# clovaai/frostnet

Measured on AMD Instinct MI355X. Metric: images/sec FrostNet-Large 224x224 QAT fwd+bwd, higher is better.
Workload: dtype int8; 1 GPU; FrostNet-Large int8 fake-quant QAT fwd+bwd + GradBoost-SGD step (noise on; StatAssist FP epoch is a one-off before it), batch=512/GPU, 224x224 NHWC, qnnpack qconfig v0 (per-tensor); per_gpu_batch=512, global_batch=512, resolution=224, parallelism=dp1, hip_graph=True, grad_dtype=bf16

## Files before the change

frostnet_amd/_lib.py:

```python
import ctypes as C
import os

import torch

_HERE = os.path.dirname(os.path.abspath(__file__))
LIB_PATH = os.environ.get("FROST_HIP_LIB", os.path.join(_HERE, "libfrost_hip.so"))
_lib = None

P, I, L, F, D = C.c_void_p, C.c_int, C.c_int64, C.c_float, C.c_double

Q_MIN, Q_MAX, Q_SCALE, Q_ZP, Q_FQMIN, Q_FQMAX, Q_INV, Q_QMAX, Q_OBS_EN, Q_FQ_EN, Q_STRIDE = 0, 1, 2, 3, 4, 5, 6, 7, 8, 10, 12
COEF_ROWS = int(os.environ.get("FROST_COEF_ROWS_ALLOC", "14"))
COEF_ROWS_NAMED = 8
DWQ_NC, DWQ_SPREAD_MAX = int(os.environ.get("FROST_DWQ_NC", "4")), 32768
COEF_A, COEF_B = 0, 1
COEF_M, COEF_R, COEF_K1, COEF_S1, COEF_S2, COEF_VFRAC = 2, 3, 4, 5, 6, 7
STATS_BYTES_PER_CH = 24 * int(os.environ.get("FROST_STATS_TABLES", "4"))


class FrostWDesc(C.Structure):
    _fields_ = [("w", P), ("gamma", P), ("rvar", P), ("qrec", P), ("wq_pack", P), ("wsum", P), ("minmax2", P),
                ("wt_pack", P), ("wscale", P), ("wmin", P), ("wmax", P), ("cout", C.c_int32), ("cin_g", C.c_int32), ("kk", C.c_int32), ("kind", C.c_int32),
                ("cpad", C.c_int32), ("kpad", C.c_int32), ("reserved0", C.c_int32), ("reserved1", C.c_int32)]

# ... 126 lines not shown
    "frost_dw_conv_fwd": [P, P, P, P, I, I, I, I, I, I, I, P, P, P, I, P, P],
    "frost_stem_im2col": [P, P, I, I, I, P, P],
    "frost_stem_wgrad_remap": [P, I, I, P, P],
    "frost_conv_finalize": [P, L, I, P, P, P, P, P, P, P, I, I, I, P, P, P, P],
    "frost_cat_observe": [P, P, P, I, P],
    "frost_cat_requant": [P, P, I, P, P, I, L, P, P, P],
    "frost_add_minmax": [P, P, P, P, L, P, P],
    "frost_add_minmax_observe": [P, P, P, P, L, P, P, I, P],
    "frost_add_requant": [P, P, P, P, L, P, P, P],
    "frost_avgpool": [P, P, I, I, I, P, P, P],
    "frost_classifier_fwd": [P, P, P, P, I, I, I, P, P, P],
    "frost_pw_conv_bwd": [P, P, P, P, P, P, L, I, I, I, P, P, I, P, P, P, I, P],
    "frost_pw_wgrad": [P, P, P, L, I, I, P, P],
    "frost_pw_bwd_fused_ok": [L, I, I],
    "frost_pw_conv_int": [P, P, P, P, L, I, I, P, P],
    "frost_pw_ew": [P, L, I, P, P, I, I, P, P, P],
    "frost_pw_ew_emit_add": [P, L, I, P, P, I, P, P, P, P, P, I, P],
    "frost_pw_ew_add_bwd": [P, L, I, P, P, I, I, P, P, P, P, P, P, I, P, P],
    "frost_pw_conv_fwd_keep": [P, P, P, P, L, I, I, P, P, P, P],
    "frost_pwc_bwd_ok": [L, I, I],
    "frost_pwc_conv_bwd": [P, P, P, P, L, I, I, I, P, P, I, P, P, P],
    "frost_pwc_conv_fwd_emit": [P, P, P, P, L, I, I, P, P, P, P],
    "frost_block_supported": [I, I, I, I, I, I],
    "frost_block_fwd": [P, P],
    "frost_block_bwd": [P, P, P],
    "frost_block_expand_dw_stats": [P, P, P, P, P, P, P, I, I, I, I, I, P, P, I, P, P, P],
    "frost_block_dw_stats": [P, P, P, P, I, I, I, I, I, P, P, P],
    "frost_block_dw_reduce_supported": [I, I, I, I, I, I],
    "frost_block_dw_bwd_supported": [I, I, I, I, I],
    "frost_block_dw_bwd_reduce": [P, P, P, P, I, I, I, I, I, P, P, I, P, P],
    "frost_block_dw_bwd": [P, P, P, P, P, P, I, I, I, I, I, P, P, I, P, P, P, P],
    "frost_block_dw_bwd_c1": [P, P, P, P, P, P, I, I, I, I, I, P, P, I, P, P, P, P, P, P, P, P, I, I, P],
    "frost_block_dw_bwd_c1_ok": [I, I, I, I, I, I],
    "frost_block_dw_reduce": [P, P, P, P, P, P, I, P, I, I, I, I, I, P, P, I, P, P, P, P],
    "frost_pw_dgrad_wide_ok": [L, I, I],
    "frost_pw_dgrad_wide": [P, P, P, L, I, I, P, I, P],
    "frost_pw_conv_bwd_fused": [P, P, P, P, P, P, L, I, I, P, P, I, P, P, P, I, P, P],
    "frost_dw_conv_bwd": [P, P, P, P, P, I, I, I, I, I, I, I, P, P, I, P, P, P],
    "frost_dw_conv_bwd_dc_wgrad": [P, P, P, P, P, I, I, I, I, I, I, P, P, I, P, P, P, P],
    "frost_dw_dgrad": [P, P, P, I, I, I, I, I, I, P, I, P, P],
    "frost_dw_wgrad": [P, P, P, I, I, I, I, I, I, P, P],
    "frost_dw_bwd_fused_ok": [I, I, I, I, I],
    "frost_dw_bwd_fused": [P, P, P, P, P, P, I, I, I, I, I, I, P, P, I, P, P, P, P],
    "frost_dw_bwd_fused_c1_ok": [I, I, I, I, I, I],
    "frost_dw_bwd_fused_c1": [P, P, P, P, P, P, I, I, I, I, I, I, P, P, I, P, P, P, P, P, P, P, P, I, I, P],
    "frost_weight_grad_finalize": [P, P, P, P, P, P, I, I, I, I, P, P, P, I, P, P],
    "frost_weight_grad_finalize_table": [P, I, P],
    "frost_infer_weight_prep": [P, I, P],
    "frost_infer_stem_im2col": [P, I, I, I, L, L, L, L, P, P],
    "frost_infer_stem_ok": [I],
    "frost_infer_stem": [P, I, I, I, L, L, L, L, P, P, I, I, P, P],
    "frost_infer_pw": [P, P, P, L, I, I, I, P, P],
    "frost_infer_dw": [P, P, P, I, I, I, I, I, I, I, P, P],
    "frost_infer_cat": [P, I, P, I, L, P, P],
    "frost_infer_add": [P, P, L, P, P],
    "frost_infer_avgpool": [P, I, I, I, P, P],
    "frost_linear_f32": [P, P, P, I, I, I, P, P],
    "frost_float_weight_prep": [P, I, P],
    "frost_float_bn_finalize": [P, I, L, P],
    "frost_float_bn_eval": [P, I, P],
    "frost_float_bwd_finalize": [P, I, L, P],
    "frost_float_pw": [P, P, P, L, I, I, I, I, P, I, P, I, P],
    "frost_float_dw": [P, P, I, I, I, I, I, I, I, I, P, P, P],
    "frost_float_ew": [P, P, L, I, I, I, P, I, P, I, P],
    "frost_float_ew_f32": [P, P, L, I, I, I, P, I, P, I, P],
    "frost_float_dw_dgrad": [P, P, I, I, I, I, I, I, P, P],
# ... 65 lines not shown
    "frost_conv_finalize_converted": [P, P, P, P, P, P, I, P, P, P],
    "frost_conv_finalize_converted_fb": [P, P, P, P, P, P, I, P, P, P],
    "frost_add_qnnpack": [P, P, P, P, L, P, P, P],
    "frost_avgpool_q": [P, I, I, I, P, P],
    "frost_cvt_head_ok": [I, I, I, I, I],
    "frost_cvt_head": [P, P, P, P, I, I, I, I, I, I, I, P, L, L, P, L, L, P],
    "frost_cvt_place": [P, P, I, I, I, I, P, L, L, P],
    "frost_stem_converted_ok": [I],
    "frost_stem_converted": [P, I, I, I, L, L, L, L, P, P, P, P, P, I, I, P, P],
    "frost_hswish_fwd": [P, P, L, P, P, P, P, I, P, P, P],
    "frost_hswish_bwd": [P, P, L, P, P, I, P],
    "frost_hswish_converted": [P, P, L, P, P, P, P, P],
    "frost_classifier_q": [P, P, P, P, I, I, I, P, P, P, P],
    "frost_classifier_q_fb": [P, P, P, P, I, I, I, P, P, P, P],
}
SYMBOLS = sorted(list(_PROTOS) + ["frost_last_error"])


def load_library():
    global _lib
    if _lib is not None:
        return _lib
    if not os.path.exists(LIB_PATH):
        raise RuntimeError(f"{LIB_PATH} not found: run `python __graft_entry__.py` (build()) first. "
                           "frostnet_amd has no CPU fallback for the HIP path.")
    lib = C.CDLL(LIB_PATH)
    for name, args in _PROTOS.items():
        fn = getattr(lib, name)
        fn.argtypes = args
        fn.restype = C.c_int
    lib.frost_last_error.restype = C.c_char_p
    lib.frost_g32_scratch_bytes.restype = C.c_int64
    lib.frost_sq_fwd_slot_bytes.restype = C.c_int64
    if lib.frost_abi_version() != ABI_VERSION or lib.frost_ticket_words() != TICKET_WORDS or lib.frost_fin_desc_bytes() != C.sizeof(FrostFinDesc):
        raise RuntimeError(f"{LIB_PATH}: ABI mismatch (library abi {lib.frost_abi_version()} / ticket words {lib.frost_ticket_words()} / FrostFinDesc "
                           f"{lib.frost_fin_desc_bytes()} B, binding {ABI_VERSION} / {TICKET_WORDS} / {C.sizeof(FrostFinDesc)} B): rebuild with `python __graft_entry__.py`")
    if lib.frost_ema_entry_bytes() != C.sizeof(FrostEmaEntry):
        raise RuntimeError(f"{LIB_PATH}: FrostEmaEntry is {lib.frost_ema_entry_bytes()} B in the library, {C.sizeof(FrostEmaEntry)} B in the binding: rebuild with `python __graft_entry__.py`")
    _lib = lib
    return lib


def ptr(t):
    if t is None:
        return None
    return C.c_void_p(t.data_ptr())


def stream():
    return C.c_void_p(torch.cuda.current_stream().cuda_stream)


class Profiler:

    def __init__(self, only=None):
        self.only = only
        self.records = []

    def summary(self):
        torch.cuda.synchronize()
        agg = {}
        for label, nbytes, e0, e1 in self.records:
            a = agg.setdefault(label, [0, 0.0, 0])
            a[0] += 1
            a[1] += e0.elapsed_time(e1)
            a[2] += nbytes
# ... 44 lines not shown
```

frostnet_amd/csrc/frost_block.hip:

```cpp
#include "frost_common.h"

typedef int v2i __attribute__((ext_vector_type(2)));
#include <stdlib.h>

__device__ __forceinline__ int blk_xcd_item(int b, int total, int on) {
  if (!on || b >= (total & ~31)) return b;
  const int xcd = b & 7, j = b >> 3;
  return (j >> 2) * 32 + xcd * 4 + (j & 3);
}
__device__ __forceinline__ int blk_xcd_run(int b, int total, int run) {
  if (run < 2 || b >= total - total % (8 * run)) return b;
  const int xcd = b & 7, j = b >> 3;
  return (j / run) * (8 * run) + xcd * run + (j % run);
}
static int blk_xcd_on() { static const int on = getenv("FROST_BLK_XCD") ? atoi(getenv("FROST_BLK_XCD")) : 1; return on; }

struct BlkAP {
  const int8_t* x; const float* qx;
  const int8_t* w1; const int32_t* wsum1;
  const float* coef1; const float* qy1; int8_t* y1;
  const int8_t* wq2; const int32_t* wsum2;
  uint8_t* stats2; FrostFinDesc fin;
  int n, cin, c, cpad, KS, kstr, nchunk, csplit, imgs, rounds, xrun;
};
// ... 1078 lines not shown
#pragma unroll
  for (int t = 0; t < K * K; ++t) red[(w * K * K + t) * 64 + lane] = (w < G::NRG) ? wacc[t] - zpf * sdc : 0.0f;
  __syncthreads();
  const float sx = p.qx[FROST_Q_SCALE];
  for (int i = tid; i < K * K * 64; i += NT) {
    const int t = i >> 6, l2 = i & 63; const int c2 = chunk * 64 + l2;
    float sum = 0.0f;
#pragma unroll
    for (int w2 = 0; w2 < NW; ++w2) sum += red[(w2 * K * K + t) * 64 + l2];
    if (c2 < p.c) atomicAdd(dwq_dst(p.dwq, (int64_t)p.c * K * K) + (int64_t)c2 * K * K + t, sum * sx);
  }
}

template <int K, int HW, int NW, int KS1 = 0>
static int launch_blk_c(BlkCP& p, hipStream_t s) {
  using G = BlkGeoC<K, HW, NW>;
  if (KS1 > 0) p.c1_kstr = KS1 * 64 + 16;
  const size_t lds = (KS1 > 0) ? (size_t)G::lds_c1(p.c1_kstr, KS1) : (size_t)G::lds();
  FROST_REQUIRE(lds <= 160 * 1024, "block_dw_bwd: LDS budget exceeded");
  static bool attr_set = false; static int occ = 0;
  if (!attr_set) {
    hipFuncSetAttribute((const void*)k_blk_dw_bwd<K, HW, NW, KS1>, hipFuncAttributeMaxDynamicSharedMemorySize, 160 * 1024); attr_set = true;
    if (hipOccupancyMaxActiveBlocksPerMultiprocessor(&occ, (const void*)k_blk_dw_bwd<K, HW, NW, KS1>, NW * 64, lds) != hipSuccess || occ < 1) occ = 1;
  }
  if (p.imgs <= 0) {
    const int rounds = p.rounds > 0 ? p.rounds : 1;
    int groups = (256 * occ * rounds) / p.nchunk; if (groups < 1) groups = 1; if (groups > p.n) groups = p.n;
    p.imgs = (p.n + groups - 1) / groups;
  }
  p.xmap = blk_xcd_on();
  hipLaunchKernelGGL((k_blk_dw_bwd<K, HW, NW, KS1>), dim3((unsigned)(((p.n + p.imgs - 1) / p.imgs) * p.nchunk)), dim3(NW * 64), lds, s, p);
  return frost_check_launch("block_dw_bwd");
}

extern "C" int frost_block_dw_bwd_supported(int h, int w, int k, int stride, int c) {
  return (h == w && (h == 7 || h == 14) && (k == 3 || k == 5) && stride == 1 && (c % 8) == 0) ? 1 : 0;
}

extern "C" int frost_block_dw_bwd_c1_ok(int h, int w, int k, int stride, int c, int c1_cin) {
  static const int on = getenv("FROST_BLK_C1") ? atoi(getenv("FROST_BLK_C1")) : 2;
  const int ks1 = (c1_cin + 63) / 64;
  return (frost_block_dw_bwd_supported(h, w, k, stride, c) && ((on >> (h == 7 ? 0 : 1)) & 1) && (c1_cin % 8) == 0 && ks1 >= 1 && ks1 <= (h == 7 ? 5 : (k == 5 ? 2 : 3))) ? 1 : 0;
}
static int blk_dw_bwd_impl(const int8_t* x, const float* qrec_x, const int8_t* wq_pack, const int32_t* wsum, const float* qrec_w, const float* wscale,
                           int n, int h, int w, int c, int k, const float* coef, const float* qrec_y, int relu, const uint16_t* gout, uint16_t* dx,
                           float* dwq, const int8_t* c1_x, const float* c1_qrec_x, const int8_t* c1_wq_pack, const int32_t* c1_wsum, float* c1_coef, int c1_cin, int c1_relu,
                           void* stream);
extern "C" int frost_block_dw_bwd(const int8_t* x, const float* qrec_x, const int8_t* wq_pack, const int32_t* wsum, const float* qrec_w, const float* wscale,
                                  int n, int h, int w, int c, int k, const float* coef, const float* qrec_y, int relu, const uint16_t* gout, uint16_t* dx,
                                  float* dwq, void* stream) {
  return blk_dw_bwd_impl(x, qrec_x, wq_pack, wsum, qrec_w, wscale, n, h, w, c, k, coef, qrec_y, relu, gout, dx, dwq, nullptr, nullptr, nullptr, nullptr, nullptr, 0, 0, stream);
}
extern "C" int frost_block_dw_bwd_c1(const int8_t* x, const float* qrec_x, const int8_t* wq_pack, const int32_t* wsum, const float* qrec_w, const float* wscale,
                                     int n, int h, int w, int c, int k, const float* coef, const float* qrec_y, int relu, const uint16_t* gout, uint16_t* dx,
                                     float* dwq, const int8_t* c1_x, const float* c1_qrec_x, const int8_t* c1_wq_pack, const int32_t* c1_wsum, float* c1_coef, int c1_cin,
                                     int c1_relu, void* stream) {
  FROST_REQUIRE(c1_x && c1_qrec_x && c1_wq_pack && c1_wsum && c1_coef && dx, "block_dw_bwd_c1: incomplete conv1 arguments (the data gradient is required)");
  FROST_REQUIRE(frost_block_dw_bwd_c1_ok(h, w, k, 1, c, c1_cin), "block_dw_bwd_c1: the conv1 fold has no instance for this shape");
  return blk_dw_bwd_impl(x, qrec_x, wq_pack, wsum, qrec_w, wscale, n, h, w, c, k, coef, qrec_y, relu, gout, dx, dwq, c1_x, c1_qrec_x, c1_wq_pack, c1_wsum, c1_coef, c1_cin, c1_relu, stream);
}
static int blk_dw_bwd_impl(const int8_t* x, const float* qrec_x, const int8_t* wq_pack, const int32_t* wsum, const float* qrec_w, const float* wscale,
                           int n, int h, int w, int c, int k, const float* coef, const float* qrec_y, int relu, const uint16_t* gout, uint16_t* dx,
                           float* dwq, const int8_t* c1_x, const float* c1_qrec_x, const int8_t* c1_wq_pack, const int32_t* c1_wsum, float* c1_coef, int c1_cin, int c1_relu,
                           void* stream) {
  FROST_REQUIRE(frost_block_dw_bwd_supported(h, w, k, 1, c), "block_dw_bwd: unsupported shape (7x7 / 14x14 maps, k in {3,5}, stride 1)");
  FROST_REQUIRE(x && wq_pack && wsum && coef && qrec_y && gout && dwq, "block_dw_bwd: incomplete arguments");
  BlkCP p = {};
  p.c1_x = c1_x; p.c1_qx = c1_qrec_x; p.c1_w = c1_wq_pack; p.c1_wsum = c1_wsum; p.c1_coef = c1_coef; p.c1_cin = c1_cin; p.c1_relu = c1_relu;
  p.x = x; p.qx = qrec_x; p.wq = wq_pack; p.wsum = wsum; p.qw = qrec_w; p.wscale = wscale; p.coef = (float*)coef ; p.qy = qrec_y; p.gout = gout; p.dx = dx; p.dwq = dwq;
  p.n = n; p.c = c; p.cpad = round_up(c, 16); p.nchunk = (c + 63) / 64; p.relu = relu; p.sr = frost_sr_enabled();
  p.inv_count = 1.0f / (float)((int64_t)n * h * w);
  static const int imgs_env = getenv("FROST_BLK_IMGS_C") ? atoi(getenv("FROST_BLK_IMGS_C")) : 0;
  static const int wgs_env = getenv("FROST_BLK_WGS_C") ? atoi(getenv("FROST_BLK_WGS_C")) : 0;
  static const int rounds_env = getenv("FROST_BLK_ROUNDS_C") ? atoi(getenv("FROST_BLK_ROUNDS_C")) : 0;
  int imgs = imgs_env > 0 ? imgs_env : (wgs_env > 0 ? (int)(((int64_t)n * p.nchunk + wgs_env - 1) / wgs_env) : 0);
  if (imgs > n) imgs = n;
  p.imgs = imgs; p.rounds = rounds_env;
  hipStream_t s = as_stream(stream);
  if (c1_x) {
    const int ks1 = (c1_cin + 63) / 64;
#define BLK_C1(KK, HH, NWW, KS) if (k == KK && h == HH && ks1 == KS) return launch_blk_c<KK, HH, NWW, KS>(p, s);
    BLK_C1(5, 7, 4, 1) BLK_C1(5, 7, 4, 2) BLK_C1(5, 7, 4, 3) BLK_C1(5, 7, 4, 4) BLK_C1(5, 7, 4, 5)
    BLK_C1(3, 7, 4, 1) BLK_C1(3, 7, 4, 2) BLK_C1(3, 7, 4, 3) BLK_C1(3, 7, 4, 4) BLK_C1(3, 7, 4, 5)
    BLK_C1(5, 14, 8, 1) BLK_C1(5, 14, 8, 2)
    BLK_C1(3, 14, 8, 1) BLK_C1(3, 14, 8, 2) BLK_C1(3, 14, 8, 3)
#undef BLK_C1
    FROST_REQUIRE(false, "block_dw_bwd_c1: no instance");
  }
  if (h == 7) return (k == 3) ? launch_blk_c<3, 7, 4>(p, s) : launch_blk_c<5, 7, 4>(p, s);
  return (k == 3) ? launch_blk_c<3, 14, 8>(p, s) : launch_blk_c<5, 14, 8>(p, s);
}

template <int K, int HW, int NW>
__global__ __launch_bounds__(NW * 64, 4) void k_blk_dw_bred(const BlkCP p) {
  using G = BlkGeoC<K, HW, NW>;
  constexpr int MAP = G::MAP, PAD = G::PAD, PITCH = G::PITCH, NT = G::NT;
  constexpr int XU = (MAP * 8 + NT - 1) / NT;
  extern __shared__ __attribute__((aligned(16))) uint8_t smem[];
  uint8_t* const xpl = smem;
  uint8_t* const gt = smem + G::PLANE;
  const int tid = threadIdx.x, lane = tid & 63, w = __builtin_amdgcn_readfirstlane(tid >> 6);
  const int bi = blk_xcd_item((int)blockIdx.x, (int)gridDim.x, p.xmap);
  const int chunk = bi % p.nchunk, ig = bi / p.nchunk;
  const int img_lo = ig * p.imgs, img_hi = min(img_lo + p.imgs, p.n);
  const int ch = chunk * 64 + lane; const bool chok = ch < p.c;
  const int zpx = __float_as_int(p.qx[FROST_Q_ZP]);
  {
    const uint32_t zf = (uint32_t)((zpx - 128) & 255) * 0x01010101u;
    for (int i = tid; i < (G::PLANE >> 4); i += NT) ((uint4*)xpl)[i] = make_uint4(zf, zf, zf, zf);
    for (int i = tid; i < (G::GT >> 4); i += NT) ((uint4*)gt)[i] = make_uint4(0, 0, 0, 0);
  }
  int wpk[K][2];
  int8_t taps[K * K];
  load_taps_i8<K * K>(p.wq, p.cpad, ch, chok, taps);
#pragma unroll
  for (int ky = 0; ky < K; ++ky) {
    uint32_t lo = 0, hi = 0;
#pragma unroll
    for (int kx = 0; kx < K; ++kx) { const uint32_t b = (uint32_t)(uint8_t)taps[ky * K + kx]; if (kx < 4) lo |= b << (8 * kx); else hi |= b; }
    wpk[ky][0] = (int)lo; wpk[ky][1] = (int)hi;
  }
// ... 209 lines not shown

template <int K, int HW, int NW>
static int launch_blk_r(BlkCP& p, hipStream_t s) {
  using G = BlkGeoC<K, HW, NW>;
  const size_t lds = (size_t)(G::PLANE + G::GT + 64);
  static bool attr_set = false; static int occ = 0;
  if (!attr_set) {
    hipFuncSetAttribute((const void*)k_blk_dw_bred<K, HW, NW>, hipFuncAttributeMaxDynamicSharedMemorySize, 160 * 1024); attr_set = true;
    if (hipOccupancyMaxActiveBlocksPerMultiprocessor(&occ, (const void*)k_blk_dw_bred<K, HW, NW>, NW * 64, lds) != hipSuccess || occ < 1) occ = 1;
  }
  if (p.imgs <= 0) {
    const int rounds = p.rounds > 0 ? p.rounds : 1;
    int groups = (256 * occ * rounds) / p.nchunk; if (groups < 1) groups = 1; if (groups > p.n) groups = p.n;
    p.imgs = (p.n + groups - 1) / groups;
  }
  p.xmap = blk_xcd_on();
  hipLaunchKernelGGL((k_blk_dw_bred<K, HW, NW>), dim3((unsigned)(((p.n + p.imgs - 1) / p.imgs) * p.nchunk)), dim3(NW * 64), lds, s, p);
  return frost_check_launch("block_dw_bwd_reduce");
}

extern "C" int frost_block_dw_bwd_reduce(const int8_t* x, const float* qrec_x, const int8_t* wq_pack, const int32_t* wsum, int n, int h, int w, int c, int k,
                                         float* coef, const float* qrec_y, int relu, const uint16_t* gout, void* stream) {
  FROST_REQUIRE((h == w && (h == 7 || h == 14) && (k == 3 || k == 5) && (c % 8) == 0), "block_dw_bwd_reduce: unsupported shape (7x7 / 14x14 maps, k in {3,5}, stride 1)");
  FROST_REQUIRE(x && wq_pack && wsum && coef && qrec_y && gout, "block_dw_bwd_reduce: incomplete arguments");
  BlkCP p = {};
  p.x = x; p.qx = qrec_x; p.wq = wq_pack; p.wsum = wsum; p.coef = coef; p.qy = qrec_y; p.gout = gout;
  p.n = n; p.c = c; p.cpad = round_up(c, 16); p.nchunk = (c + 63) / 64; p.relu = relu;
  static const int wgs_env = getenv("FROST_BLK_WGS_R") ? atoi(getenv("FROST_BLK_WGS_R")) : 0;
  static const int rounds_env = getenv("FROST_BLK_ROUNDS_R") ? atoi(getenv("FROST_BLK_ROUNDS_R")) : 2;
  int imgs = wgs_env > 0 ? (int)(((int64_t)n * p.nchunk + wgs_env - 1) / wgs_env) : 0;
  if (imgs > n) imgs = n;
  p.imgs = imgs; p.rounds = rounds_env;
  hipStream_t s = as_stream(stream);
  if (h == 7) return (k == 3) ? launch_blk_r<3, 7, 4>(p, s) : launch_blk_r<5, 7, 4>(p, s);
  return (k == 3) ? launch_blk_r<3, 14, 8>(p, s) : launch_blk_r<5, 14, 8>(p, s);
}

extern "C" int frost_block_supported(int h, int w, int k, int stride, int cin, int c) {
  return (h == w && (h == 7 || h == 14) && (k == 3 || k == 5) && stride == 1 && (cin % 8) == 0 && cin > (h == 7 ? 64 : 0) && cin <= (h == 7 ? 320 : 192) && (c % 8) == 0) ? 1 : 0;
}

extern "C" int frost_block_expand_dw_stats(const int8_t* x, const float* qrec_x, const int8_t* w1_pack, const int32_t* wsum1, const float* coef1,
                                           const float* qrec_y1, int8_t* y1, int n, int h, int w, int cin, int c, const int8_t* wq2,
                                           const int32_t* wsum2, int k, void* stats2, const FrostFinDesc* fin2, void* stream) {
  FROST_REQUIRE(frost_block_supported(h, w, k, 1, cin, c), "block_expand_dw: unsupported shape (7x7 / 14x14 maps, k in {3,5}, stride 1, cin <= 320 / 192)");
  FROST_REQUIRE(fin2 && fin2->counter && fin2->coef && fin2->qrec_y, "block_expand_dw: incomplete finalize descriptor");
  BlkAP p = {};
  p.x = x; p.qx = qrec_x; p.w1 = w1_pack; p.wsum1 = wsum1; p.coef1 = coef1; p.qy1 = qrec_y1; p.y1 = y1; p.wq2 = wq2; p.wsum2 = wsum2;
  p.stats2 = (uint8_t*)stats2; p.fin = *fin2; p.n = n; p.cin = cin; p.c = c; p.cpad = round_up(c, 16); p.KS = (cin + 63) / 64; p.kstr = p.KS * 64 + 16;
  p.nchunk = (c + 63) / 64;
  static const int cpw_env = getenv("FROST_BLK_CPW") ? atoi(getenv("FROST_BLK_CPW")) : 0, imgs_env = getenv("FROST_BLK_IMGS") ? atoi(getenv("FROST_BLK_IMGS")) : 0;
  int cpw = cpw_env > 0 ? cpw_env : 2;
  if (cpw > p.nchunk) cpw = p.nchunk;
  p.csplit = (p.nchunk + cpw - 1) / cpw;
  static const int rounds_env = getenv("FROST_BLK_ROUNDS_A") ? atoi(getenv("FROST_BLK_ROUNDS_A")) : 0;
  p.imgs = imgs_env > 0 ? imgs_env : 0;
  p.rounds = rounds_env > 0 ? rounds_env : (h == 14 ? 2 : 1);
  hipStream_t s = as_stream(stream);
#define BLK_A(KK, HH, NWW, KSS) if (k == KK && h == HH && p.KS == KSS) return launch_blk_a<KK, HH, NWW, KSS>(p, s);
  BLK_A(3, 7, 4, 2) BLK_A(3, 7, 4, 3) BLK_A(3, 7, 4, 4) BLK_A(3, 7, 4, 5) BLK_A(5, 7, 4, 2) BLK_A(5, 7, 4, 3) BLK_A(5, 7, 4, 4) BLK_A(5, 7, 4, 5)
  BLK_A(3, 14, 8, 1) BLK_A(3, 14, 8, 2) BLK_A(3, 14, 8, 3) BLK_A(5, 14, 8, 1) BLK_A(5, 14, 8, 2) BLK_A(5, 14, 8, 3)
#undef BLK_A
  FROST_REQUIRE(false, "block_expand_dw: no instance");
  return 1;
}

// ... 576 lines not shown
```

include/frost_hip.h:

```cpp
#ifndef FROST_HIP_H
#define FROST_HIP_H
#include <stdint.h>

#ifdef __cplusplus
extern "C" {
#endif

#ifndef FROST_DWQ_NC
#define FROST_DWQ_NC 4
#endif
#define FROST_DWQ_SPREAD_MAX 32768
#define FROST_ABI_VERSION 5

#define FROST_Q_MIN 0
#define FROST_Q_MAX 1
#define FROST_Q_SCALE 2
#define FROST_Q_ZP 3
#define FROST_Q_FQMIN 4
#define FROST_Q_FQMAX 5
#define FROST_Q_INV 6
#define FROST_Q_QMAX 7
#define FROST_Q_OBS_EN 8
#define FROST_Q_FQ_EN 10
#define FROST_Q_STRIDE 12
// ... 329 lines not shown
                          int stride, void* stats, const FrostFinDesc* fin, void* stream);
int frost_pw_conv_fwd_keep(const int8_t* x, const float* qrec_x, const int8_t* wq_pack, const int32_t* wsum, int64_t npix, int cin, int cout,
                           void* stats, const FrostFinDesc* fin, int32_t* conv_out, void* stream);

int frost_pw_ew_add_bwd(const int32_t* conv_out, int64_t npix, int cout, float* coef, const float* qrec_y, int relu, int mode, const uint16_t* gsum,
                        const int8_t* a, const float* qrec_a, const int8_t* yb, const float* qrec_sum, uint16_t* ga, int acc_a, uint16_t* dc, void* stream);
int frost_pw_ew_emit_add(const int32_t* conv_out, int64_t npix, int cout, const float* coef, const float* qrec_y, int relu, const int8_t* a,
                         const float* qrec_a, int8_t* y, float* state3, float* qrec_sum, int observe, void* stream);

int frost_pwc_bwd_ok(int64_t npix, int cin, int cout);
int frost_pwc_conv_fwd_emit(const int8_t* x, const float* qrec_x, const int8_t* wq_pack, const int32_t* wsum, int64_t npix, int cin, int cout,
                            const float* coef, const float* qrec_y, int8_t* y, void* stream);
int frost_pwc_conv_bwd(const int8_t* x, const float* qrec_x, const int8_t* wq_pack, const int32_t* wsum, int64_t npix, int cin, int cout, int pass,
                       float* coef, const float* qrec_y, int relu, const uint16_t* gout, uint16_t* dc, void* stream);

int frost_block_supported(int h, int w, int k, int stride, int cin, int c);
int frost_block_dw_stats(const int8_t* x, const float* qrec_x, const int8_t* wq_pack, const int32_t* wsum, int n, int h, int w, int c, int k, void* stats,
                         const FrostFinDesc* fin, void* stream);
int frost_block_expand_dw_stats(const int8_t* x, const float* qrec_x, const int8_t* w1_pack, const int32_t* wsum1, const float* coef1,
                                const float* qrec_y1, int8_t* y1, int n, int h, int w, int cin, int c, const int8_t* wq2, const int32_t* wsum2,
                                int k, void* stats2, const FrostFinDesc* fin2, void* stream);

int frost_block_dw_reduce_supported(int h, int w, int k, int stride, int c, int cout);
int frost_block_dw_reduce(const int8_t* y1, const float* qrec_y1, const int8_t* wq2, const int32_t* wsum2, const float* coef2, const float* qrec_y2,
                          int relu2, int8_t* y2, int n, int h, int w, int c, int k, const int8_t* w3_pack, const int32_t* wsum3, int cout,
                          int32_t* conv_out, void* stats3, const FrostFinDesc* fin3, void* stream);

int frost_block_dw_bwd_supported(int h, int w, int k, int stride, int c);
int frost_block_dw_bwd_reduce(const int8_t* x, const float* qrec_x, const int8_t* wq_pack, const int32_t* wsum, int n, int h, int w, int c, int k,
                              float* coef, const float* qrec_y, int relu, const uint16_t* gout, void* stream);
int frost_block_dw_bwd(const int8_t* x, const float* qrec_x, const int8_t* wq_pack, const int32_t* wsum, const float* qrec_w, const float* wscale,
                       int n, int h, int w, int c, int k, const float* coef, const float* qrec_y, int relu, const uint16_t* gout, uint16_t* dx,
                       float* dwq, void* stream);
int frost_block_dw_bwd_c1_ok(int h, int w, int k, int stride, int c, int c1_cin);
int frost_block_dw_bwd_c1(const int8_t* x, const float* qrec_x, const int8_t* wq_pack, const int32_t* wsum, const float* qrec_w, const float* wscale,
                          int n, int h, int w, int c, int k, const float* coef, const float* qrec_y, int relu, const uint16_t* gout, uint16_t* dx,
                          float* dwq, const int8_t* c1_x, const float* c1_qrec_x, const int8_t* c1_wq_pack, const int32_t* c1_wsum, float* c1_coef, int c1_cin,
                          int c1_relu, void* stream);

typedef struct {
  const int8_t* wq_pack; const int32_t* wsum; void* stats; FrostFinDesc fin;
  const uint16_t* wt_pack; float* dwq;
  int32_t cout, k;
} FrostBlockLayer;
typedef struct {
  int32_t n, h, w, cin;
  const int8_t* x; const float* qrec_x;
  FrostBlockLayer conv1, conv2, reduce;
  int8_t* y1; int8_t* y2; int32_t* conv_out3; int8_t* y3;
} FrostBlockDesc;
typedef struct {
  const uint16_t* gout3;
  uint16_t* dc3; uint16_t* g2; uint16_t* g1; uint16_t* dc1;
  uint16_t* dx;
  void* side_stream;
} FrostBlockBwd;
int frost_block_fwd(const FrostBlockDesc* d, void* stream);
int frost_block_bwd(const FrostBlockDesc* d, const FrostBlockBwd* b, void* stream);

int frost_softmax_ce(const float* logits, const int64_t* target, int n, int c, float inv_n, float* loss, float* dlogits, void* stream);
int frost_softmax_ce_metrics(const float* logits, const int64_t* target, int n, int c, float inv_n, int topk, float* loss, float* dlogits,
                             double* record, void* stream);
int frost_dropout_mask(void* draw_counter, uint64_t seed, int64_t n, float keep, float* out, void* stream);

int frost_conv_finalize_converted(const float* qrec_x, const float* qrec_w, const float* gamma, const float* beta,
                                  const float* rmean, const float* rvar, int cout, float* coef, const float* qrec_y, void* stream);
// ... 162 lines not shown
```

Measured before the change: 26720 images/sec.

## Add wave-per-image kernels for 7x7 depthwise backward and reduce passes

Measured after the change: 26940 images/sec (median of 6 runs). Within noise of the previous version (+0.8%).

```diff
diff --git a/frostnet_amd/_lib.py b/frostnet_amd/_lib.py
--- a/frostnet_amd/_lib.py
+++ b/frostnet_amd/_lib.py
@@ -182,6 +182,8 @@
     "frost_block_dw_bwd": [P, P, P, P, P, P, I, I, I, I, I, P, P, I, P, P, P, P],
     "frost_block_dw_bwd_c1": [P, P, P, P, P, P, I, I, I, I, I, P, P, I, P, P, P, P, P, P, P, P, I, I, P],
     "frost_block_dw_bwd_c1_ok": [I, I, I, I, I, I],
+    "frost_block_dw_wave7_set": [I],
+    "frost_block_dw_wave7_get": [],
     "frost_block_dw_reduce": [P, P, P, P, P, P, I, P, I, I, I, I, I, P, P, I, P, P, P, P],
     "frost_pw_dgrad_wide_ok": [L, I, I],
     "frost_pw_dgrad_wide": [P, P, P, L, I, I, P, I, P],
@@ -313,6 +315,7 @@
     lib.frost_last_error.restype = C.c_char_p
     lib.frost_g32_scratch_bytes.restype = C.c_int64
     lib.frost_sq_fwd_slot_bytes.restype = C.c_int64
+    lib.frost_block_dw_wave7_set.restype = None
     if lib.frost_abi_version() != ABI_VERSION or lib.frost_ticket_words() != TICKET_WORDS or lib.frost_fin_desc_bytes() != C.sizeof(FrostFinDesc):
         raise RuntimeError(f"{LIB_PATH}: ABI mismatch (library abi {lib.frost_abi_version()} / ticket words {lib.frost_ticket_words()} / FrostFinDesc "
                            f"{lib.frost_fin_desc_bytes()} B, binding {ABI_VERSION} / {TICKET_WORDS} / {C.sizeof(FrostFinDesc)} B): rebuild with `python __graft_entry__.py`")
diff --git a/frostnet_amd/csrc/frost_block.hip b/frostnet_amd/csrc/frost_block.hip
--- a/frostnet_amd/csrc/frost_block.hip
+++ b/frostnet_amd/csrc/frost_block.hip
@@ -1134,6 +1134,335 @@
   hipLaunchKernelGGL((k_blk_dw_bwd<K, HW, NW, KS1>), dim3((unsigned)(((p.n + p.imgs - 1) / p.imgs) * p.nchunk)), dim3(NW * 64), lds, s, p);
   return frost_check_launch("block_dw_bwd");
 }
+
+static int blk_wave7_env() { static const int on = getenv("FROST_BLK_WAVE7") ? atoi(getenv("FROST_BLK_WAVE7")) : 1; return on; }
+static int g_blk_wave7 = -1;
+extern "C" void frost_block_dw_wave7_set(int on) { g_blk_wave7 = (on < 0) ? -1 : (on ? 1 : 0); }
+extern "C" int frost_block_dw_wave7_get(void) { return (g_blk_wave7 >= 0) ? g_blk_wave7 : (blk_wave7_env() ? 1 : 0); }
+
+__device__ __forceinline__ void blk_wsync() { asm volatile("s_waitcnt lgkmcnt(0)" ::: "memory"); __builtin_amdgcn_wave_barrier(); }
+
+constexpr int BLK_W7_XT = 50 * 64, BLK_W7_TILE = BLK_W7_XT + 50 * 128, BLK_W7_NU = 7;
+
+struct BlkW7Stage {
+  uint2 xv[BLK_W7_NU]; uint4 gv[BLK_W7_NU];
+  int vo, vo6; bool pok;
+  __device__ __forceinline__ void init(const BlkCP& p, int chunk, int lane) {
+    const int part = lane & 7;
+    pok = (chunk * 64 + part * 8) < p.c;
+    vo6 = chunk * 64 + (pok ? part * 8 : 0);
+    vo = (lane >> 3) * p.c + vo6;
+  }
+  __device__ __forceinline__ void load(const BlkCP& p, int img) {
+    const int8_t* xs = p.x + (int64_t)img * 49 * p.c;
+    const uint16_t* gs = p.gout + (int64_t)img * 49 * p.c;
+#pragma unroll
+    for (int i = 0; i < BLK_W7_NU; ++i) {
+      const int o = (i < BLK_W7_NU - 1) ? vo : vo6;
+      xv[i] = *(const uint2*)(xs + (int64_t)(8 * i) * p.c + o);
+      gv[i] = *(const uint4*)(gs + (int64_t)(8 * i) * p.c + o);
+    }
+  }
+  __device__ __forceinline__ void store(uint8_t* xt, uint8_t* gt, int lane) const {
+#pragma unroll
+    for (int i = 0; i < BLK_W7_NU; ++i) {
+      if (i < BLK_W7_NU - 1 || lane < 8) {
+        *(uint2*)(xt + (lane + 64 * i) * 8) = pok ? xv[i] : make_uint2(0, 0);
+        *(uint4*)(gt + (lane + 64 * i) * 16) = pok ? gv[i] : make_uint4(0, 0, 0, 0);
+      }
+    }
+  }
+};
+
+template <int K, typename F>
+__device__ __forceinline__ void blk_w7_conv(const uint8_t* xt, int lane, uint32_t zpfill, const int (&wpk)[K][2], const int (&rsz)[K], F&& row_done) {
+  constexpr int PAD = (K - 1) / 2, NWIN = (K == 3) ? 7 : 11;
+  int acc[7][7];
+#pragma unroll
+  for (int iy = 0; iy < 7; ++iy) {
+    const v2i a = blk_tr8(xt, iy * 7, lane);
+    int dd[4];
+    if (K == 5) {
+      dd[0] = (int)__builtin_amdgcn_perm((uint32_t)a[0], zpfill, 0x05040000u);
+      dd[1] = (int)__builtin_amdgcn_alignbyte((uint32_t)a[1], (uint32_t)a[0], 2);
+      dd[2] = (int)__builtin_amdgcn_perm((uint32_t)a[1], zpfill, 0x00000006u);
+    } else {
+      dd[0] = (int)__builtin_amdgcn_perm((uint32_t)a[0], zpfill, 0x06050400u);
+      dd[1] = (int)__builtin_amdgcn_alignbyte((uint32_t)a[1], (uint32_t)a[0], 3);
+      dd[2] = (int)zpfill;
+    }
+    dd[3] = 0;
+    int win[NWIN];
+#pragma unroll
+    for (int i = 0; i < NWIN; ++i) win[i] = (i % 4 == 0) ? dd[i / 4] : (int)__builtin_amdgcn_alignbyte((uint32_t)dd[i / 4 + 1], (uint32_t)dd[i / 4], i % 4);
+#pragma unroll
+    for (int ky = K - 1; ky >= 0; --ky) {
+      const int oy = iy + PAD - ky;
+      if (oy >= 0 && oy < 7) {
+        if (iy == ((oy - PAD > 0) ? oy - PAD : 0)) {
+          int a0 = 0;
+#pragma unroll
+          for (int k2 = 0; k2 < K; ++k2) if (oy + k2 - PAD >= 0 && oy + k2 - PAD < 7) a0 += rsz[k2];
+#pragma unroll
+          for (int ox = 0; ox < 7; ++ox) acc[oy][ox] = a0;
+        }
+#pragma unroll
+        for (int ox = 0; ox < 7; ++ox) {
+          acc[oy][ox] = __builtin_amdgcn_sdot4(win[ox], wpk[ky][0], acc[oy][ox], false);
+          if (K == 5) acc[oy][ox] = __builtin_amdgcn_sdot4(win[ox + 4], wpk[ky][1], acc[oy][ox], false);
+        }
+      }
+    }
+    __builtin_amdgcn_sched_barrier(0);
+    if (iy - PAD >= 0) { row_done(iy - PAD, acc[iy - PAD]); __builtin_amdgcn_sched_barrier(0); }
+  }
+#pragma unroll
+  for (int oy = 7 - PAD; oy < 7; ++oy) { row_done(oy, acc[oy]); __builtin_amdgcn_sched_barrier(0); }
+}
+
+template <int K>
+__device__ __forceinline__ void blk_w7_taps(const BlkCP& p, int ch, bool chok, int zpx, int8_t (&taps)[K * K], int (&wpk)[K][2], int (&rsz)[K]) {
+  load_taps_i8<K * K>(p.wq, p.cpad, ch, chok, taps);
+#pragma unroll
+  for (int ky = 0; ky < K; ++ky) {
+    uint32_t lo = 0, hi = 0; int rs = 0;
+#pragma unroll
+    for (int kx = 0; kx < K; ++kx) { const uint32_t b = (uint32_t)(uint8_t)taps[ky * K + kx]; rs += (int)taps[ky * K + kx]; if (kx < 4) lo |= b << (8 * kx); else hi |= b; }
+    wpk[ky][0] = (int)lo; wpk[ky][1] = (int)hi; rsz[ky] = (128 - zpx) * rs;
+  }
+}
+
+template <int K>
+__global__ __launch_bounds__(256, 2) void k_blk_dw_bwd_w7(const BlkCP p) {
+  constexpr int MAP = 49, PAD = (K - 1) / 2, NW = 4, NT = 256, NPW = (K + 1) / 2;
+  extern __shared__ __attribute__((aligned(16))) uint8_t smem[];
+  const int tid = threadIdx.x, lane = tid & 63, w = __builtin_amdgcn_readfirstlane(tid >> 6);
+  uint8_t* const xt = smem + w * BLK_W7_TILE;
+  uint8_t* const gt = xt + BLK_W7_XT;
+  const int bi = blk_xcd_item((int)blockIdx.x, (int)gridDim.x, p.xmap);
+  const int chunk = bi % p.nchunk, ig = bi / p.nchunk;
+  const int img_lo = ig * p.imgs, img_hi = min(img_lo + p.imgs, p.n);
+  const int ch = chunk * 64 + lane; const bool chok = ch < p.c;
+  const int zpx = __float_as_int(p.qx[FROST_Q_ZP]);
+  const uint32_t zpfill = (uint32_t)((zpx - 128) & 255) * 0x01010101u;
+  const float zpf = (float)zpx;
+  int wpk[K][2], rsz[K]; int8_t taps[K * K];
+  blk_w7_taps<K>(p, ch, chok, zpx, taps, wpk, rsz);
+  uint32_t wp2[K][NPW];
+#pragma unroll
+  for (int ky = 0; ky < K; ++ky)
+#pragma unroll
+    for (int a = 0; a < NPW; ++a) {
+      const uint32_t hi = __float_as_uint((float)taps[ky * K + 2 * a]) >> 16;
+      const uint32_t lo = (2 * a + 1 < K) ? (__float_as_uint((float)taps[ky * K + 2 * a + 1]) >> 16) : 0u;
+      wp2[ky][a] = (2 * a + 1 < K) ? (lo | (hi << 16)) : hi;
+    }
+  const float sw = (p.wscale && chok) ? p.wscale[ch] : p.qw[FROST_Q_SCALE];
+  float cA = 0, cB = 0, cK1 = 0, cE = 0, cF = 0;
+  if (chok) {
+    cA = p.coef[FROST_COEF_A * p.cpad + ch]; cB = p.coef[FROST_COEF_B * p.cpad + ch];
+    const float m = p.coef[FROST_COEF_M * p.cpad + ch], cR = p.coef[FROST_COEF_R * p.cpad + ch];
+    cK1 = p.coef[FROST_COEF_K1 * p.cpad + ch];
+    cE = -cK1 * (s12_sum(p.coef, p.cpad, 1, ch) * p.inv_count) * cR;
+    cF = -cK1 * (s12_sum(p.coef, p.cpad, 0, ch) * p.inv_count) - cE * m;
+  }
+  const float y_inv = 1.0f / p.qy[FROST_Q_SCALE];
+  float t_lo = 0.0f, t_hi;
+  {
+    const int zpy = __float_as_int(p.qy[FROST_Q_ZP]), qhi = q_hi(p.qy);
+    const float hi0 = (float)qhi + 0.5f - (float)zpy;
+    t_hi = ((qhi - zpy) & 1) ? __int_as_float(__float_as_int(hi0) - 1) : hi0;
+    if (!p.relu) { const float lo0 = -(float)zpy - 0.5f; t_lo = (zpy & 1) ? lo0 : __int_as_float(__float_as_int(lo0) + 1); }
+  }
+  uint32_t rng = sr_seed(blockIdx.x, threadIdx.x);
+  const bool sr_on = p.sr != 0;
+  float wacc[K * K];
+#pragma unroll
+  for (int t = 0; t < K * K; ++t) wacc[t] = 0.0f;
+  BlkW7Stage st; st.init(p, chunk, lane);
+  if (img_lo + w < img_hi) st.load(p, img_lo + w);
+
+  for (int img = img_lo + w; img < img_hi; img += NW) {
+    st.store(xt, gt, lane);
+    if (img + NW < img_hi) st.load(p, img + NW);
+    blk_wsync();
+    uint32_t E[7][4];
+    blk_w7_conv<K>(xt, lane, zpfill, wpk, rsz, [&](int oy, const int (&a)[7]) __attribute__((always_inline)) {
+      uint32_t g2[4];
+      blk_tr16_raw(gt, oy * 7, lane, g2); blk_tr16_raw(gt, oy * 7 + 4, lane, g2 + 2);
+      uint32_t hb[8]; hb[7] = 0u;
+#pragma unroll
+      for (int r = 0; r < 7; ++r) {
+        const float gq = __uint_as_float((r & 1) ? (g2[r >> 1] & 0xffff0000u) : (g2[r >> 1] << 16));
+        const float v = (float)a[r];
+        const float tq = fmaf(cA, v, cB) * y_inv;
+        const float gy = (chok && tq > t_lo && tq <= t_hi) ? gq : 0.0f;
+        const float dcf = fmaf(gy, cK1, fmaf(v, cE, cF));
+        const uint32_t db = __float_as_uint(dcf), dr = sr_next16(rng);
+        hb[r] = chok ? ((db + (sr_on ? dr : 0x7fffu + ((db >> 16) & 1u))) >> 16) : 0u;
+      }
+#pragma unroll
+      for (int j = 0; j < 4; ++j) E[oy][j] = hb[2 * j] | (hb[2 * j + 1] << 16);
+    });
+#pragma unroll
+    for (int iy = 0; iy < 7; ++iy) {
+      const v2i ra = blk_tr8(xt, iy * 7, lane);
+      const uint32_t u[2] = {(uint32_t)ra[0] ^ 0x80808080u, (uint32_t)ra[1] ^ 0x80808080u};
+      float xf[9]; xf[0] = 0.0f; xf[8] = 0.0f;
+#pragma unroll
+      for (int i = 0; i < 7; ++i) xf[i + 1] = (float)((u[i >> 2] >> (8 * (i & 3))) & 255u) - zpf;
+      uint32_t X2[8];
+#pragma unroll
+      for (int i = 0; i < 8; ++i) X2[i] = __builtin_amdgcn_perm(__float_as_uint(xf[i + 1]), __float_as_uint(xf[i]), 0x07060302u);
+#pragma unroll
+      for (int ky = 0; ky < K; ++ky) {
+        const int oy = iy + PAD - ky;
+        if (oy >= 0 && oy < 7) {
+#pragma unroll
+          for (int kx = 0; kx < K; ++kx)
+#pragma unroll
+            for (int r2 = 0; r2 < 4; ++r2) {
+              const int s = 2 * r2 + kx - PAD;
+              if (s >= -1 && s <= 6) wacc[ky * K + kx] = blk_dot2(E[oy][r2], X2[s + 1], wacc[ky * K + kx]);
+            }
+        }
+      }
+      __builtin_amdgcn_sched_barrier(0);
+    }
+    if (p.dx) {
+      float acc[7][7];
+#pragma unroll
+      for (int r = 0; r < 7; ++r) {
+        uint32_t O[4];
+        O[0] = E[r][0] << 16;
+#pragma unroll
+        for (int j = 1; j < 4; ++j) O[j] = __builtin_amdgcn_alignbit(E[r][j], E[r][j - 1], 16);
+#pragma unroll
+        for (int ky = K - 1; ky >= 0; --ky) {
+          const int iy = r - PAD + ky;
+          if (iy >= 0 && iy < 7) {
+            if (r == ((iy - PAD > 0) ? iy - PAD : 0)) {
+#pragma unroll
+              for (int ix = 0; ix < 7; ++ix) acc[iy][ix] = 0.0f;
+            }
+#pragma unroll
+            for (int ix = 0; ix < 7; ++ix)
+#pragma unroll
+              for (int a = 0; a < NPW; ++a) {
+                const int s = ((2 * a + 1 < K) ? ix + K - 2 - 2 * a : ix) - PAD;
+                if (s >= -1 && s <= 6) acc[iy][ix] = blk_dot2((s & 1) ? O[(s + 1) >> 1] : E[r][s >> 1], wp2[ky][a], acc[iy][ix]);
+              }
+          }
+        }
+        __builtin_amdgcn_sched_barrier(0);
+#pragma unroll
+        for (int iy = r - PAD; iy <= ((r == 6) ? 6 : r - PAD); ++iy) {
+          if (iy >= 0) {
+            uint16_t* dst = p.dx + ((int64_t)img * MAP + iy * 7) * p.c;
+#pragma unroll
+            for (int ix = 0; ix < 7; ++ix) {
+              const float dxv = acc[iy][ix] * sw;
+              if (chok) dst[(int64_t)ix * p.c + ch] = (uint16_t)cvt_pk_bf16(dxv, 0.0f);
+            }
+          }
+        }
+        __builtin_amdgcn_sched_barrier(0);
+      }
+    }
+    blk_wsync();
+  }
+  __syncthreads();
+  float* red = (float*)smem;
+#pragma unroll
+  for (int t = 0; t < K * K; ++t) red[(w * K * K + t) * 64 + lane] = wacc[t];
+  __syncthreads();
+  const float sx = p.qx[FROST_Q_SCALE];
+  for (int i = tid; i < K * K * 64; i += NT) {
+    const int t = i >> 6, l2 = i & 63; const int c2 = chunk * 64 + l2;
+    float sum = 0.0f;
+#pragma unroll
+    for (int w2 = 0; w2 < NW; ++w2) sum += red[(w2 * K * K + t) * 64 + l2];
+    if (c2 < p.c) atomicAdd(dwq_dst(p.dwq, (int64_t)p.c * K * K) + (int64_t)c2 * K * K + t, sum * sx);
+  }
+}
+
+template <int K>
+__global__ __launch_bounds__(256, (K == 3) ? 4 : 3) void k_blk_dw_bred_w7(const BlkCP p) {
+  constexpr int NW = 4;
+  extern __shared__ __attribute__((aligned(16))) uint8_t smem[];
+  const int tid = threadIdx.x, lane = tid & 63, w = __builtin_amdgcn_readfirstlane(tid >> 6);
+  uint8_t* const xt = smem + w * BLK_W7_TILE;
+  uint8_t* const gt = xt + BLK_W7_XT;
+  const int bi = blk_xcd_item((int)blockIdx.x, (int)gridDim.x, p.xmap);
+  const int chunk = bi % p.nchunk, ig = bi / p.nchunk;
+  const int img_lo = ig * p.imgs, img_hi = min(img_lo + p.imgs, p.n);
+  const int ch = chunk * 64 + lane; const bool chok = ch < p.c;
+  const int zpx = __float_as_int(p.qx[FROST_Q_ZP]);
+  const uint32_t zpfill = (uint32_t)((zpx - 128) & 255) * 0x01010101u;
+  int wpk[K][2], rsz[K]; int8_t taps[K * K];
+  blk_w7_taps<K>(p, ch, chok, zpx, taps, wpk, rsz);
+  float cA = 0, cB = 0, cR = 0, cMR = 0;
+  if (chok) {
+    cA = p.coef[FROST_COEF_A * p.cpad + ch]; cB = p.coef[FROST_COEF_B * p.cpad + ch];
+    cR = p.coef[FROST_COEF_R * p.cpad + ch]; cMR = -p.coef[FROST_COEF_M * p.cpad + ch] * cR;
+  }
+  const float y_inv = 1.0f / p.qy[FROST_Q_SCALE];
+  float t_lo = 0.0f, t_hi;
+  {
+    const int zpy = __float_as_int(p.qy[FROST_Q_ZP]), qhi = q_hi(p.qy);
+    const float hi0 = (float)qhi + 0.5f - (float)zpy;
+    t_hi = ((qhi - zpy) & 1) ? __int_as_float(__float_as_int(hi0) - 1) : hi0;
+    if (!p.relu) { const float lo0 = -(float)zpy - 0.5f; t_lo = (zpy & 1) ? lo0 : __int_as_float(__float_as_int(lo0) + 1); }
+  }
+  float r1 = 0.0f, r2 = 0.0f;
+  BlkW7Stage st; st.init(p, chunk, lane);
+  if (img_lo + w < img_hi) st.load(p, img_lo + w);
+  for (int img = img_lo + w; img < img_hi; img += NW) {
+    st.store(xt, gt, lane);
+    if (img + NW < img_hi) st.load(p, img + NW);
+    blk_wsync();
+    blk_w7_conv<K>(xt, lane, zpfill, wpk, rsz, [&](int oy, const int (&a)[7]) __attribute__((always_inline)) {
+      uint32_t g2[4];
+      blk_tr16_raw(gt, oy * 7, lane, g2); blk_tr16_raw(gt, oy * 7 + 4, lane, g2 + 2);
+#pragma unroll
+      for (int r = 0; r < 7; ++r) {
+        const float gq = __uint_as_float((r & 1) ? (g2[r >> 1] & 0xffff0000u) : (g2[r >> 1] << 16));
+        const float v = (float)a[r];
+        const float tq = fmaf(cA, v, cB) * y_inv;
+        const float gy = (chok && tq > t_lo && tq <= t_hi) ? gq : 0.0f;
+        r1 += gy; r2 = fmaf(gy, fmaf(v, cR, cMR), r2);
+      }
+    });
+    blk_wsync();
+  }
+  __syncthreads();
+  float* red = (float*)smem;
+  red[(w * 2) * 64 + lane] = r1; red[(w * 2 + 1) * 64 + lane] = r2;
+  __syncthreads();
+  if (tid < 128) {
+    const int which = tid >> 6, l2 = tid & 63, c2 = chunk * 64 + l2;
+    float sum = 0.0f;
+#pragma unroll
+    for (int w2 = 0; w2 < NW; ++w2) sum += red[(w2 * 2 + which) * 64 + l2];
+    if (c2 < p.c) atomicAdd(s12_dst(p.coef, p.cpad, which) + c2, sum);
+  }
+}
+
+template <typename KernT>
+static int launch_blk_w7(KernT kern, BlkCP& p, int& occ, const char* what, hipStream_t s) {
+  const size_t lds = (size_t)4 * BLK_W7_TILE;
+  if (occ == 0 && (hipOccupancyMaxActiveBlocksPerMultiprocessor(&occ, (const void*)kern, 256, lds) != hipSuccess || occ < 1)) occ = 1;
+  if (p.imgs <= 0) {
+    const int rounds = p.rounds > 0 ? p.rounds : 1;
+    int groups = (256 * occ * rounds) / p.nchunk; if (groups < 1) groups = 1; if (groups > p.n) groups = p.n;
+    p.imgs = (p.n + groups - 1) / groups;
+  }
+  p.xmap = blk_xcd_on();
+  hipLaunchKernelGGL(kern, dim3((unsigned)(((p.n + p.imgs - 1) / p.imgs) * p.nchunk)), dim3(256), lds, s, p);
+  return frost_check_launch(what);
+}
+template <int K> static int launch_blk_c7(BlkCP& p, hipStream_t s) { static int occ = 0; return launch_blk_w7(k_blk_dw_bwd_w7<K>, p, occ, "block_dw_bwd", s); }
+template <int K> static int launch_blk_r7(BlkCP& p, hipStream_t s) { static int occ = 0; return launch_blk_w7(k_blk_dw_bred_w7<K>, p, occ, "block_dw_bwd_reduce", s); }
 
 extern "C" int frost_block_dw_bwd_supported(int h, int w, int k, int stride, int c) {
   return (h == w && (h == 7 || h == 14) && (k == 3 || k == 5) && stride == 1 && (c % 8) == 0) ? 1 : 0;
@@ -1189,6 +1518,7 @@
 #undef BLK_C1
     FROST_REQUIRE(false, "block_dw_bwd_c1: no instance");
   }
+  if (h == 7 && frost_block_dw_wave7_get()) return (k == 3) ? launch_blk_c7<3>(p, s) : launch_blk_c7<5>(p, s);
   if (h == 7) return (k == 3) ? launch_blk_c<3, 7, 4>(p, s) : launch_blk_c<5, 7, 4>(p, s);
   return (k == 3) ? launch_blk_c<3, 14, 8>(p, s) : launch_blk_c<5, 14, 8>(p, s);
 }
@@ -1464,6 +1794,7 @@
   if (imgs > n) imgs = n;
   p.imgs = imgs; p.rounds = rounds_env;
   hipStream_t s = as_stream(stream);
+  if (h == 7 && frost_block_dw_wave7_get()) return (k == 3) ? launch_blk_r7<3>(p, s) : launch_blk_r7<5>(p, s);
   if (h == 7) return (k == 3) ? launch_blk_r<3, 7, 4>(p, s) : launch_blk_r<5, 7, 4>(p, s);
   return (k == 3) ? launch_blk_r<3, 14, 8>(p, s) : launch_blk_r<5, 14, 8>(p, s);
 }
diff --git a/include/frost_hip.h b/include/frost_hip.h
--- a/include/frost_hip.h
+++ b/include/frost_hip.h
@@ -385,6 +385,8 @@
 int frost_block_dw_bwd(const int8_t* x, const float* qrec_x, const int8_t* wq_pack, const int32_t* wsum, const float* qrec_w, const float* wscale,
                        int n, int h, int w, int c, int k, const float* coef, const float* qrec_y, int relu, const uint16_t* gout, uint16_t* dx,
                        float* dwq, void* stream);
+void frost_block_dw_wave7_set(int on);
+int frost_block_dw_wave7_get(void);
 int frost_block_dw_bwd_c1_ok(int h, int w, int k, int stride, int c, int c1_cin);
 int frost_block_dw_bwd_c1(const int8_t* x, const float* qrec_x, const int8_t* wq_pack, const int32_t* wsum, const float* qrec_w, const float* wscale,
                           int n, int h, int w, int c, int k, const float* coef, const float* qrec_y, int relu, const uint16_t* gout, uint16_t* dx,
```
